# JackShDr/InfluentialRS

Hardware: NVIDIA B200
Metric: IRN influence-path generation throughput @1M items (higher is better)
Workload: dtype f32

## Files before the change

### influentialrs_b200/csrc/decoder_chain_tc.cu

```cuda
#include "tc_common.cuh"
#include "qkv_image.cuh"

namespace irs {
namespace tcl {

using namespace irs::tc;

constexpr int BM = 128, D = 128, F = 256;
constexpr int RING = 4;
constexpr uint32_t UNIT_BYTES = 16384, UNIT_HALF = 8192;
constexpr uint32_t A_LBO = BM * 16;
constexpr uint32_t SBO = 128;
constexpr uint32_t OFF_P = 0;
constexpr uint32_t OFF_Q = 65536;
constexpr uint32_t OFF_RING = 131072;
constexpr uint32_t OFF_VEC = OFF_RING + RING * UNIT_BYTES;
constexpr int V_BO = 0, V_G1 = 128, V_B1 = 256, V_C2 = 384, V_G2 = 512, V_B2 = 640, V_BF1 = 768, V_BF2 = 1024,
              V_G3 = 1152, V_B3 = 1280, V_BIN = 1408, V_TOTAL = 1792;
constexpr uint32_t OFF_XCH = OFF_VEC + V_TOTAL * 4;
constexpr uint32_t OFF_BARS = OFF_XCH + 3 * 2 * 128 * 8;
enum Bars { B_FULL = 0, B_EMPTY = 4, B_A0 = 8, B_D1 = 9, B_A1 = 10, B_D2 = 11, B_A2 = 12 , B_D3 = 16,
            B_A3 = 17, B_D4 = 18, B_COUNT = 20 };
constexpr uint32_t OFF_TMEM = OFF_BARS + B_COUNT * 8;
constexpr uint32_t SMEM_BYTES = OFF_TMEM + 16;
constexpr int EPI_WARPS = 8, EPI_THREADS = EPI_WARPS * 32;
constexpr int LOAD_WARPS = 2;
constexpr int WARP_LOAD0 = 8, WARP_PROD = 10, WARP_MMA = 11;
constexpr int THREADS = 12 * 32;
constexpr int UNITS_BODY = 20;
constexpr int UNITS_QKV = 12;
constexpr uint32_t T_H = 0, T_Y = 256, T_D3 = 384;

struct Params {
  const float* attn;
  const float* x;
  float* x_out;
  float* qkv_out;
  uint8_t* qkv_images;
  int L, mask_mode;
  int qkv_only;
  const uint4* wstream;
  const float* vec[11];
  float eps1, eps2, eps3;
  int64_t R; int64_t n_tiles; int n_units;
  int* error_flag;
  long long* timeline;
};

struct UnitDesc { int mat, n0, k0, kind; };
__host__ __device__ inline UnitDesc unit_desc(int u) {
  UnitDesc d;
  if (u < 4) { d.mat = 0; d.n0 = 0; d.k0 = 32 * u; d.kind = 0; }
  else if (u < 12) { d.mat = 1; d.n0 = 0; d.k0 = 16 * (u - 4); d.kind = 2; }
  else if (u < 20) { d.mat = 2; d.n0 = 0; d.k0 = 32 * (u - 12); d.kind = 0; }
  else if (u < 28) { d.mat = 3; d.n0 = 0; d.k0 = 16 * (u - 20); d.kind = 2; }
  else { d.mat = 3; d.n0 = 256; d.k0 = 32 * (u - 28); d.kind = 0; }
  return d;
}

__global__ void __launch_bounds__(256)
prepare_chain_kernel(const float* __restrict__ Wo, const float* __restrict__ W1, const float* __restrict__ W2,
                     const float* __restrict__ Win, int n_units, uint4* __restrict__ out) {
  const int total = n_units * 1024;
  for (int idx = blockIdx.x * blockDim.x + threadIdx.x; idx < total; idx += gridDim.x * blockDim.x) {
    const int u = idx >> 10, w = idx & 1023;
    const int part = w >> 9, rem = w & 511;
    const UnitDesc ud = unit_desc(u);
    int slab, row;
    if (ud.kind == 0) { slab = rem >> 7; row = rem & 127; } else { slab = rem >> 8; row = rem & 255; }
    const float* W; int ldw;
    switch (ud.mat) { case 0: W = Wo; ldw = D; break; case 1: W = W1; ldw = D; break; case 2: W = W2; ldw = F; break;
                      default: W = Win; ldw = D; break; }
    const float* src = W + (int64_t)(ud.n0 + row) * ldw + ud.k0 + slab * 8;
    float x[8];
#pragma unroll
    for (int e = 0; e < 8; ++e) x[e] = src[e];
    uint4 hi, lo;
    split8(x, hi, lo);
    out[idx] = part ? lo : hi;
  }
}

__device__ __forceinline__ void ldg256_nc(const float* p, float (&a)[8]) {
  asm volatile("ld.global.nc.L1::no_allocate.v8.f32 {%0,%1,%2,%3,%4,%5,%6,%7}, [%8];"
               : "=f"(a[0]), "=f"(a[1]), "=f"(a[2]), "=f"(a[3]), "=f"(a[4]), "=f"(a[5]), "=f"(a[6]), "=f"(a[7]) : "l"(p));
}
__device__ __forceinline__ void ldg256(const float* p, float (&a)[8]) {
  asm volatile("ld.global.L1::no_allocate.v8.f32 {%0,%1,%2,%3,%4,%5,%6,%7}, [%8];"
               : "=f"(a[0]), "=f"(a[1]), "=f"(a[2]), "=f"(a[3]), "=f"(a[4]), "=f"(a[5]), "=f"(a[6]), "=f"(a[7]) : "l"(p) : "memory");
}
__device__ __forceinline__ void stg256(float* p, const float* a) {
  asm volatile("st.global.L1::no_allocate.v8.f32 [%0], {%1,%2,%3,%4,%5,%6,%7,%8};"
               :: "l"(p), "f"(a[0]), "f"(a[1]), "f"(a[2]), "f"(a[3]), "f"(a[4]), "f"(a[5]), "f"(a[6]), "f"(a[7]) : "memory");
}
__device__ __forceinline__ void stg128(void* p, const uint4& v) {
  asm volatile("st.global.L1::no_allocate.v4.b32 [%0], {%1,%2,%3,%4};" :: "l"(p), "r"(v.x), "r"(v.y), "r"(v.z), "r"(v.w) : "memory");
}
__device__ __forceinline__ void prefetch_l2_bulk(const void* p, uint32_t bytes) {
  asm volatile("cp.async.bulk.prefetch.L2.global [%0], %1;" :: "l"(p), "r"(bytes) : "memory");
}

template <int KSTEPS>
__device__ __forceinline__ void mma_unit(uint32_t d_tmem, uint32_t a_hi, uint32_t a_lo, uint32_t b_stage, uint32_t b_lbo,
                                         uint32_t idesc, bool first) {
#pragma unroll
  for (int kk = 0; kk < KSTEPS; ++kk) {
    const uint64_t ah = make_desc(a_hi + (uint32_t)(2 * kk) * A_LBO, A_LBO, SBO);
    const uint64_t al = make_desc(a_lo + (uint32_t)(2 * kk) * A_LBO, A_LBO, SBO);
    const uint64_t bh = make_desc(b_stage + (uint32_t)(2 * kk) * b_lbo, b_lbo, SBO);
    const uint64_t bl = make_desc(b_stage + UNIT_HALF + (uint32_t)(2 * kk) * b_lbo, b_lbo, SBO);
    tc_mma_bf16(d_tmem, al, bh, idesc, (first && kk == 0) ? 0u : 1u);
    tc_mma_bf16(d_tmem, ah, bl, idesc, 1u);
    tc_mma_bf16(d_tmem, ah, bh, idesc, 1u);
  }
}

#define IRS_TL(role, idx)                                                                         \
  do {                                                                                            \
    if (p.timeline && blockIdx.x == 0 && it < 8 && lane == 0)                                     \
      p.timeline[(it * 3 + (role)) * 32 + (idx)] = clock64();                                     \
  } while (0)

__device__ __forceinline__ void pair_barrier(int quad) {
  asm volatile("bar.sync %0, 64;" :: "r"(1 + quad) : "memory");
}

__device__ __forceinline__ float2 ln_pair_stats(float (&t)[64], float2* mine, const float2* other, int quad, float eps) {
  float s[4] = {0.f, 0.f, 0.f, 0.f}, q[4] = {0.f, 0.f, 0.f, 0.f};
#pragma unroll
  for (int j = 0; j < 64; ++j) s[j & 3] += t[j];
  const float m = ((s[0] + s[1]) + (s[2] + s[3])) * (1.0f / 64.0f);
#pragma unroll
  for (int j = 0; j < 64; ++j) {
    t[j] -= m;
    q[j & 3] = fmaf(t[j], t[j], q[j & 3]);
  }
  const float qs = (q[0] + q[1]) + (q[2] + q[3]);
  *mine = make_float2(m, qs);
  pair_barrier(quad);
  const float2 o = *other;
  const float delta = o.x - m;
  const float mean = 0.5f * (m + o.x);
  const float rstd = rsqrtf(fmaf(32.f * delta, delta, qs + o.y) * (1.0f / (float)D) + eps);
  return make_float2(rstd, (m - mean) * rstd);
}

__global__ void __launch_bounds__(THREADS, 1)
decoder_chain_kernel(const Params p) {
  extern __shared__ __align__(128) uint8_t smem[];
  const uint32_t sbase = smem_u32(smem);
  const int tid = threadIdx.x, warp = tid >> 5, lane = tid & 31;
  auto bar = [&](int i) { return sbase + OFF_BARS + 8u * (uint32_t)i; };
  volatile uint32_t* tmem_holder = reinterpret_cast<volatile uint32_t*>(smem + OFF_TMEM);
  float* vecs = reinterpret_cast<float*>(smem + OFF_VEC);
  const bool with_qkv = (p.qkv_out != nullptr) || (p.qkv_images != nullptr);
  const bool qkv_only = p.qkv_only != 0;

  if (tid == 0) {
    for (int s = 0; s < RING; ++s) { mbar_init(bar(B_FULL + s), 1); mbar_init(bar(B_EMPTY + s), 1); }
    mbar_init(bar(B_A0), LOAD_WARPS);
    mbar_init(bar(B_D1), 1);
    mbar_init(bar(B_A1), EPI_THREADS);
    mbar_init(bar(B_D2), 1);
    for (int i = 0; i < 4; ++i) mbar_init(bar(B_A2 + i), EPI_THREADS);
    mbar_init(bar(B_D3), 1);
    mbar_init(bar(B_A3), EPI_THREADS);
    for (int i = 0; i < 2; ++i) mbar_init(bar(B_D4 + i), 1);
    asm volatile("fence.mbarrier_init.release.cluster;" ::: "memory");
  }
  if (warp == WARP_MMA) {
    asm volatile("tcgen05.alloc.cta_group::1.sync.aligned.shared::cta.b32 [%0], %1;" :: "r"(sbase + OFF_TMEM), "r"(512u) : "memory");
    asm volatile("tcgen05.relinquish_alloc_permit.cta_group::1.sync.aligned;" ::: "memory");
  }
  {
    const int vlen[11] = {128, 128, 128, 128, 128, 128, 256, 128, 128, 128, 384};
    int off = 0;
    const float qscale0 = 1.4426950408889634f / sqrtf((float)img::DH);
    for (int v = 0; v < 11; ++v) {
      for (int i = tid; i < vlen[v]; i += THREADS) {
        float x = p.vec[v] ? p.vec[v][i] : 0.f;
        if (v == 2 && p.vec[3]) x += p.vec[3][i];
        if (v == 10 && p.qkv_images && i < D) x *= qscale0;
        vecs[off + i] = x;
      }
      off += vlen[v];
    }
  }
  tc_fence_before();
  __syncthreads();
  tc_fence_after();
  const uint32_t tmem_base = *tmem_holder;
  const int64_t first_tile = blockIdx.x, tile_step = gridDim.x;

  if (warp >= WARP_LOAD0 && warp < WARP_LOAD0 + LOAD_WARPS) {
    const int lw = warp - WARP_LOAD0;
    const int r8 = lane & 7, sg = lane >> 3;
    const uint32_t a0_off = qkv_only ? OFF_P : OFF_Q;
    int it = 0;
    for (int64_t tile = first_tile; tile < p.n_tiles; tile += tile_step, ++it) {
      const int64_t r0 = tile * BM;
#pragma unroll 1
      for (int batch = 0; batch < 64 / LOAD_WARPS / 8; ++batch) {
        float v[8][8];
#pragma unroll
        for (int q = 0; q < 8; ++q) {
          const int qq = batch * 8 + q;
          const int row = (lw * (16 / LOAD_WARPS) + (qq >> 2)) * 8 + r8;
          const int slab = (qq & 3) * 4 + sg;
          if (r0 + row < p.R) ldg256_nc(p.attn + (r0 + row) * D + slab * 8, v[q]);
          else {
#pragma unroll
            for (int e = 0; e < 8; ++e) v[q][e] = 0.f;
          }
        }
        if (batch == 0 && lw == 0) IRS_TL(2, 0);
        if (batch == 0 && it > 0) mbar_wait(bar(qkv_only ? B_D4 + 1 : B_D3), (uint32_t)((it - 1) & 1), p.error_flag, 31);
        if (batch == 0 && lw == 0) IRS_TL(2, 1);
#pragma unroll
        for (int q = 0; q < 8; ++q) {
          const int qq = batch * 8 + q;
          const int row = (lw * (16 / LOAD_WARPS) + (qq >> 2)) * 8 + r8;
          const int slab = (qq & 3) * 4 + sg;
          uint4 hi, lo;
          split8(v[q], hi, lo);
          *reinterpret_cast<uint4*>(smem + a0_off + slab * A_LBO + row * 16) = hi;
          *reinterpret_cast<uint4*>(smem + a0_off + 32768 + slab * A_LBO + row * 16) = lo;
        }
      }
      asm volatile("fence.proxy.async.shared::cta;" ::: "memory");
      __syncwarp();
      if (lane == 0) mbar_arrive(bar(B_A0));
      if (lw == 0) IRS_TL(2, 2);
    }
  } else if (warp == WARP_PROD) {
    if (lane == 0) {
      int64_t g = 0;
      for (int64_t tile = first_tile; tile < p.n_tiles; tile += tile_step) {
        const int64_t nt = tile + tile_step;
        if (nt < p.n_tiles) {
          const int64_t rows = (p.R - nt * BM) < BM ? (p.R - nt * BM) : BM;
          if (p.x) prefetch_l2_bulk(p.x + nt * BM * D, (uint32_t)(rows * D * 4));
          prefetch_l2_bulk(p.attn + nt * BM * D, (uint32_t)(rows * D * 4));
        }
        for (int u = 0; u < p.n_units; ++u, ++g) {
          const int stage = (int)(g % RING);
          const uint32_t phase = (uint32_t)((g / RING) & 1);
          mbar_wait(bar(B_EMPTY + stage), phase ^ 1u, p.error_flag, 32);
          mbar_arrive_expect_tx(bar(B_FULL + stage), UNIT_BYTES);
          bulk_g2s(sbase + OFF_RING + stage * UNIT_BYTES, p.wstream + (int64_t)u * (UNIT_BYTES / 16), UNIT_BYTES, bar(B_FULL + stage));
        }
      }
    }
  } else if (warp == WARP_MMA) {
    if (lane == 0) {
      const uint32_t idesc128 = make_idesc_bf16(BM, 128), idesc256 = make_idesc_bf16(BM, 256);
      const uint32_t P_HI = sbase + OFF_P, P_LO = sbase + OFF_P + 32768, Q_HI = sbase + OFF_Q, Q_LO = sbase + OFF_Q + 32768;
      int64_t g = 0;
      auto next_unit = [&]() -> uint32_t {
        const int stage = (int)(g % RING);
        mbar_wait(bar(B_FULL + stage), (uint32_t)((g / RING) & 1), p.error_flag, 33);
        tc_fence_after();
        return sbase + OFF_RING + stage * UNIT_BYTES;
      };
      auto release_unit = [&]() { tc_commit(bar(B_EMPTY + (int)(g % RING))); ++g; };
      int it = 0;
      for (int64_t tile = first_tile; tile < p.n_tiles; tile += tile_step, ++it) {
        const uint32_t ph = (uint32_t)(it & 1);
        if (qkv_only) {
          mbar_wait(bar(B_A0), ph, p.error_flag, 34);
          if (it > 0) mbar_wait(bar(B_A1), (uint32_t)((it - 1) & 1), p.error_flag, 38);
          tc_fence_after();
          for (int u = 0; u < 8; ++u) {
            const uint32_t bs = next_unit();
            mma_unit<1>(tmem_base + T_H, P_HI + (uint32_t)(2 * u) * A_LBO, P_LO + (uint32_t)(2 * u) * A_LBO, bs, 4096u, idesc256, u == 0);
            release_unit();
          }
          tc_commit(bar(B_D4 + 0));
          for (int c = 0; c < 4; ++c) {
            const uint32_t bs = next_unit();
            mma_unit<2>(tmem_base + T_D3, P_HI + (uint32_t)(4 * c) * A_LBO, P_LO + (uint32_t)(4 * c) * A_LBO, bs, 2048u, idesc128, c == 0);
            release_unit();
          }
          tc_commit(bar(B_D4 + 1));
          continue;
        }
        IRS_TL(0, 0);
        mbar_wait(bar(B_A0), ph, p.error_flag, 34);
        tc_fence_after();
        IRS_TL(0, 1);
        for (int c = 0; c < 4; ++c) {
          const uint32_t bs = next_unit();
          mma_unit<2>(tmem_base + T_Y, Q_HI + (uint32_t)(4 * c) * A_LBO, Q_LO + (uint32_t)(4 * c) * A_LBO, bs, 2048u, idesc128, c == 0);
          release_unit();
        }
        tc_commit(bar(B_D1));
        IRS_TL(0, 2);
        mbar_wait(bar(B_A1), ph, p.error_flag, 35);
        tc_fence_after();
        IRS_TL(0, 3);
        for (int u = 0; u < 8; ++u) {
          const uint32_t bs = next_unit();
          mma_unit<1>(tmem_base + T_H, P_HI + (uint32_t)(2 * u) * A_LBO, P_LO + (uint32_t)(2 * u) * A_LBO, bs, 4096u, idesc256, u == 0);
          release_unit();
        }
        tc_commit(bar(B_D2));
        for (int j = 0; j < 4; ++j) {
          IRS_TL(0, 4 + 2 * j);
          mbar_wait(bar(B_A2 + j), ph, p.error_flag, 36);
          tc_fence_after();
          IRS_TL(0, 5 + 2 * j);
          const uint32_t slot = (j < 2 ? Q_HI : P_HI) + (uint32_t)(j & 1) * 32768u;
          for (int i = 0; i < 2; ++i) {
            const uint32_t bs = next_unit();
            mma_unit<2>(tmem_base + T_D3, slot + (uint32_t)(4 * i) * A_LBO, slot + 16384u + (uint32_t)(4 * i) * A_LBO, bs,
                        2048u, idesc128, j == 0 && i == 0);
            release_unit();
          }
        }
        tc_commit(bar(B_D3));
        IRS_TL(0, 12);
        mbar_wait(bar(B_A3), ph, p.error_flag, 37);
        tc_fence_after();
        IRS_TL(0, 13);
        if (with_qkv) {
          for (int u = 0; u < 8; ++u) {
            const uint32_t bs = next_unit();
            mma_unit<1>(tmem_base + T_H, P_HI + (uint32_t)(2 * u) * A_LBO, P_LO + (uint32_t)(2 * u) * A_LBO, bs, 4096u, idesc256, u == 0);
            release_unit();
          }
          tc_commit(bar(B_D4 + 0));
          IRS_TL(0, 14);
          for (int c = 0; c < 4; ++c) {
            const uint32_t bs = next_unit();
            mma_unit<2>(tmem_base + T_D3, P_HI + (uint32_t)(4 * c) * A_LBO, P_LO + (uint32_t)(4 * c) * A_LBO, bs, 2048u, idesc128, c == 0);
            release_unit();
          }
          tc_commit(bar(B_D4 + 1));
          IRS_TL(0, 15);
        }
      }
    }
  } else if (warp < EPI_WARPS) {
    const int quad = warp & 3, half = warp >> 2;
    const int row = quad * 32 + lane;
    const uint32_t tlane = tmem_base + (((uint32_t)(quad * 32)) << 16);
    float2* xch = reinterpret_cast<float2*>(smem + OFF_XCH);
    const int c0 = half * 64;
    auto e4_piece = [&](int64_t tile, int it, int piece) {
      const uint32_t ph = (uint32_t)(it & 1);
      const int64_t r = tile * BM + row;
      const bool row_ok = r < p.R;
      float* qo = p.qkv_out ? p.qkv_out + (row_ok ? r : 0) * (3 * D) : nullptr;
      const int bb = (int)(r / p.L), ll = (int)(r - (int64_t)bb * p.L);
      const int n_chunks = (p.L + 31) / 32;
      const int qs = img::q_slot(n_chunks, ll);
      const uint32_t q_off = img::OFF_Q + (uint32_t)(qs / BM) * img::Q_TILE + (uint32_t)(qs % BM) * 16u;
      const uint32_t kv_off = (uint32_t)img::kv_col(p.mask_mode == IRS_MASK_PIM, p.L, ll) * 16u;
      uint8_t* item0 = p.qkv_images ? p.qkv_images + (int64_t)bb * (D / img::DH) * img::ITEM_BYTES : nullptr;
      const float qscale = 1.4426950408889634f / sqrtf((float)img::DH);
      {
      mbar_wait(bar(B_D4 + piece), ph, p.error_flag, 45);
      tc_fence_after();
      if (warp == 0) IRS_TL(1, 13 + 2 * piece);
      const int ncol = piece == 0 ? 128 : 64;
      const int col0 = piece == 0 ? half * 128 : 256 + half * 64;
      const uint32_t tcol = piece == 0 ? (T_H + (uint32_t)half * 128u) : (T_D3 + (uint32_t)half * 64u);
      auto emit = [&](const uint32_t (&v)[32], int ch) {
        float o32[32];
        const float sc = (p.qkv_images && col0 + ch * 32 < D) ? qscale : 1.0f;
#pragma unroll
        for (int j = 0; j < 32; ++j) o32[j] = fmaf(__uint_as_float(v[j]), sc, vecs[V_BIN + col0 + ch * 32 + j]);
        if (qo) {
          if (row_ok) {
#pragma unroll
            for (int q = 0; q < 4; ++q) stg256(qo + col0 + ch * 32 + q * 8, &o32[q * 8]);
          }
        } else if (row_ok) {
          const int c = col0 + ch * 32;
          const int which = c >> 7, head = (c & 127) >> 5;
          uint8_t* dst = item0 + (int64_t)head * img::ITEM_BYTES + (which == 0 ? q_off : (which == 1 ? img::OFF_K : img::OFF_V) + kv_off);
          const uint32_t lbo = which == 0 ? img::Q_LBO : img::K_LBO, part = which == 0 ? img::Q_PART : img::K_PART;
#pragma unroll
          for (int s8 = 0; s8 < 4; ++s8) {
            uint4 hi, lo;
            split8(*reinterpret_cast<float(*)[8]>(&o32[s8 * 8]), hi, lo);
            stg128(dst + s8 * lbo, hi);
            stg128(dst + part + s8 * lbo, lo);
          }
        }
      };
      {
        const int nch = ncol / 32;
        uint32_t va[32], vb[32];
        tc_ld32(tlane + tcol, va);
#pragma unroll 1
        for (int ch = 0; ch < nch; ch += 2) {
          tc_wait_ld();
          if (ch + 1 < nch) tc_ld32(tlane + tcol + (ch + 1) * 32, vb);
          emit(va, ch);
          if (ch + 1 < nch) {
            tc_wait_ld();
            if (ch + 2 < nch) tc_ld32(tlane + tcol + (ch + 2) * 32, va);
            emit(vb, ch + 1);
          }
        }
      }
      if (warp == 0) IRS_TL(1, 14 + 2 * piece);
      }
    };
    int it = 0;
    for (int64_t tile = first_tile; tile < p.n_tiles; tile += tile_step, ++it) {
      const uint32_t ph = (uint32_t)(it & 1);
      const int64_t r = tile * BM + row;
      const bool row_ok = r < p.R;
      if (!qkv_only) {
      float t[64];
      {
        const float* xrow = p.x + (row_ok ? r : 0) * D + c0;
#pragma unroll
        for (int q = 0; q < 8; ++q) {
          if (row_ok) ldg256(xrow + q * 8, *reinterpret_cast<float(*)[8]>(&t[q * 8]));
          else {
#pragma unroll
            for (int e = 0; e < 8; ++e) t[q * 8 + e] = 0.f;
          }
        }
      }
      if (warp == 0) IRS_TL(1, 0);
      mbar_wait(bar(B_D1), ph, p.error_flag, 41);
      tc_fence_after();
      if (warp == 0) IRS_TL(1, 1);
#pragma unroll
      for (int ch = 0; ch < 2; ++ch) {
        uint32_t v[32];
        tc_ld32(tlane + T_Y + c0 + ch * 32, v);
        tc_wait_ld();
#pragma unroll
        for (int j = 0; j < 32; ++j) {
          t[ch * 32 + j] = __uint_as_float(v[j]) + vecs[V_BO + c0 + ch * 32 + j] + t[ch * 32 + j];
        }
      }
      const float2 st1 = ln_pair_stats(t, &xch[(0 * 2 + half) * 128 + row], &xch[(0 * 2 + (half ^ 1)) * 128 + row],
                                       quad, p.eps1);
#pragma unroll
      for (int j = 0; j < 64; ++j) {
        const int n = c0 + j;
        t[j] = fmaf(fmaf(t[j], st1.x, st1.y), vecs[V_G1 + n], vecs[V_B1 + n]);
      }
      const float2 st2 = ln_pair_stats(t, &xch[(1 * 2 + half) * 128 + row], &xch[(1 * 2 + (half ^ 1)) * 128 + row],
                                       quad, p.eps2);
#pragma unroll
      for (int ch = 0; ch < 2; ++ch) {
        uint32_t v[32];
#pragma unroll
        for (int j = 0; j < 32; ++j) {
          const int n = c0 + ch * 32 + j;
          const float y = fmaf(fmaf(t[ch * 32 + j], st2.x, st2.y), vecs[V_G2 + n], vecs[V_B2 + n]);
          t[ch * 32 + j] = y;
          v[j] = __float_as_uint(y);
        }
        tc_st32(tlane + T_Y + c0 + ch * 32, v);
#pragma unroll
        for (int s8 = 0; s8 < 4; ++s8) {
          uint4 hi, lo;
          split8(*reinterpret_cast<float(*)[8]>(&t[ch * 32 + s8 * 8]), hi, lo);
          const uint32_t o = (uint32_t)(half * 8 + ch * 4 + s8) * A_LBO + (uint32_t)row * 16u;
          *reinterpret_cast<uint4*>(smem + OFF_P + o) = hi;
          *reinterpret_cast<uint4*>(smem + OFF_P + 32768 + o) = lo;
        }
      }
      tc_wait_st();
      asm volatile("fence.proxy.async.shared::cta;" ::: "memory");
      tc_fence_before();
      mbar_arrive(bar(B_A1));
      if (warp == 0) IRS_TL(1, 2);
      if (with_qkv && it > 0) e4_piece(tile - tile_step, it - 1, 1);
      mbar_wait(bar(B_D2), ph, p.error_flag, 42);
      tc_fence_after();
#pragma unroll 1
      for (int j = 0; j < 4; ++j) {
        uint32_t v[32];
        tc_ld32(tlane + T_H + 64u * (uint32_t)j + 32u * (uint32_t)half, v);
        if (warp == 0) IRS_TL(1, 3 + 2 * j);
        uint8_t* slot = smem + (j < 2 ? OFF_Q : OFF_P) + (j & 1) * 32768;
        tc_wait_ld();
#pragma unroll
        for (int s8 = 0; s8 < 4; ++s8) {
          float x8[8];
#pragma unroll
          for (int e = 0; e < 8; ++e)
            x8[e] = fmaxf(__uint_as_float(v[s8 * 8 + e]) + vecs[V_BF1 + j * 64 + half * 32 + s8 * 8 + e], 0.f);
          uint4 hi, lo;
          split8(x8, hi, lo);
          const uint32_t o = (uint32_t)(half * 4 + s8) * A_LBO + (uint32_t)row * 16u;
          *reinterpret_cast<uint4*>(slot + o) = hi;
          *reinterpret_cast<uint4*>(slot + 16384 + o) = lo;
        }
        asm volatile("fence.proxy.async.shared::cta;" ::: "memory");
        tc_fence_before();
        mbar_arrive(bar(B_A2 + j));
        if (warp == 0) IRS_TL(1, 4 + 2 * j);
      }
      mbar_wait(bar(B_D3), ph, p.error_flag, 44);
      tc_fence_after();
      if (warp == 0) IRS_TL(1, 11);
#pragma unroll
      for (int ch = 0; ch < 2; ++ch) {
        uint32_t v[32], y[32];
        tc_ld32(tlane + T_D3 + c0 + ch * 32, v);
        tc_ld32(tlane + T_Y + c0 + ch * 32, y);
        tc_wait_ld();
#pragma unroll
        for (int j = 0; j < 32; ++j) {
          t[ch * 32 + j] = __uint_as_float(v[j]) + vecs[V_BF2 + c0 + ch * 32 + j] + __uint_as_float(y[j]);
        }
      }
      const float2 st3 = ln_pair_stats(t, &xch[(2 * 2 + half) * 128 + row], &xch[(2 * 2 + (half ^ 1)) * 128 + row],
                                       quad, p.eps3);
      float* xo = p.x_out + (row_ok ? r : 0) * D + c0;
#pragma unroll
      for (int ch = 0; ch < 2; ++ch) {
#pragma unroll
        for (int j = 0; j < 32; ++j) {
          const int n = c0 + ch * 32 + j;
          t[ch * 32 + j] = fmaf(fmaf(t[ch * 32 + j], st3.x, st3.y), vecs[V_G3 + n], vecs[V_B3 + n]);
        }
        if (row_ok) {
#pragma unroll
          for (int q = 0; q < 4; ++q) stg256(xo + ch * 32 + q * 8, &t[ch * 32 + q * 8]);
        }
        if (with_qkv) {
#pragma unroll
          for (int s8 = 0; s8 < 4; ++s8) {
            uint4 hi, lo;
            split8(*reinterpret_cast<float(*)[8]>(&t[ch * 32 + s8 * 8]), hi, lo);
            const uint32_t o = (uint32_t)(half * 8 + ch * 4 + s8) * A_LBO + (uint32_t)row * 16u;
            *reinterpret_cast<uint4*>(smem + OFF_P + o) = hi;
            *reinterpret_cast<uint4*>(smem + OFF_P + 32768 + o) = lo;
          }
        }
      }
      if (with_qkv) asm volatile("fence.proxy.async.shared::cta;" ::: "memory");
      tc_fence_before();
      mbar_arrive(bar(B_A3));
      if (warp == 0) IRS_TL(1, 12);
      }
      if (qkv_only) {
        e4_piece(tile, it, 0);
        e4_piece(tile, it, 1);
        tc_fence_before();
        mbar_arrive(bar(B_A1));
      } else if (with_qkv) {
        e4_piece(tile, it, 0);
      }
      tc_fence_before();
    }
    if (!qkv_only && with_qkv && it > 0) e4_piece(first_tile + (int64_t)(it - 1) * tile_step, it - 1, 1);
    tc_fence_before();
  }

  tc_fence_before();
  __syncthreads();
  if (warp == WARP_MMA) {
    tc_fence_after();
    asm volatile("tcgen05.dealloc.cta_group::1.sync.aligned.b32 %0, %1;" :: "r"(tmem_base), "r"(512u) : "memory");
  }
}

}
}

using namespace irs;

static long long* g_chain_timeline = nullptr;

extern "C" void irs_decoder_chain_debug_timeline(long long* buf) { g_chain_timeline = buf; }

extern "C" int irs_decoder_chain_supported(int d, int ffn) { return (d == tcl::D && ffn == tcl::F) ? 1 : 0; }

extern "C" size_t irs_decoder_chain_prepared_bytes(int d, int ffn, int with_in_proj) {
  if (!irs_decoder_chain_supported(d, ffn)) return 0;
  return (size_t)(tcl::UNITS_BODY + (with_in_proj ? tcl::UNITS_QKV : 0)) * tcl::UNIT_BYTES;
}

extern "C" int irs_decoder_chain_prepare_weights(const float* Wo, const float* W1, const float* W2, const float* Win,
                                                 int d, int ffn, void* prepared, void* stream) {
  if (!Wo || !W1 || !W2 || !prepared) return IRS_E_BADARG;
  if (!irs_decoder_chain_supported(d, ffn)) return IRS_E_SHAPE;
  const int n_units = tcl::UNITS_BODY + (Win ? tcl::UNITS_QKV : 0);
  tcl::prepare_chain_kernel<<<64, 256, 0, (cudaStream_t)stream>>>(Wo, W1, W2, Win, n_units, (uint4*)prepared);
  IRS_LAUNCHED();
  return 0;
}

static int chain_launch(tcl::Params& p, int64_t R, int* error_flag, void* stream) {
  p.R = R; p.n_tiles = ceil_div(R, tcl::BM);
  p.error_flag = error_flag;
  p.timeline = g_chain_timeline;
  static bool configured = false;
  if (!configured) {
    IRS_CUDA(cudaFuncSetAttribute(tcl::decoder_chain_kernel, cudaFuncAttributeMaxDynamicSharedMemorySize, (int)tcl::SMEM_BYTES));
    configured = true;
  }
  const unsigned grid = (unsigned)(p.n_tiles < kNumSMs ? p.n_tiles : kNumSMs);
  tcl::decoder_chain_kernel<<<grid, tcl::THREADS, tcl::SMEM_BYTES, (cudaStream_t)stream>>>(p);
  IRS_LAUNCHED();
  return 0;
}

extern "C" int irs_decoder_chain_tc(const float* attn, const float* x, const void* prepared,
                                    const float* bo, const float* g1, const float* b1, const float* c2,
                                    const float* g2, const float* b2, const float* bf1, const float* bf2,
                                    const float* g3, const float* b3, const float* bin,
                                    float eps1, float eps2, float eps3,
                                    float* x_out, float* qkv_out, void* qkv_images, int L, int mask_mode,
                                    int64_t R, int d, int ffn, int* error_flag, void* stream) {
  if (!attn || !x || !prepared || !x_out || !g1 || !b1 || !g2 || !b2 || !g3 || !b3) return IRS_E_BADARG;
  if (R < 0 || (qkv_out && qkv_images)) return IRS_E_BADARG;
  if (R == 0) return 0;
  if (!irs_decoder_chain_supported(d, ffn)) return IRS_E_SHAPE;
  if (qkv_images && (L <= 128 || L > irs::img::KEYS - 1 || R % L != 0 || mask_mode < 0 || mask_mode > 2)) return IRS_E_SHAPE;
  if (((uintptr_t)attn & 31) || ((uintptr_t)x & 31) || ((uintptr_t)x_out & 31) || ((uintptr_t)qkv_out & 31) ||
      ((uintptr_t)qkv_images & 15) || ((uintptr_t)prepared & 15))
    return IRS_E_SHAPE;
  tcl::Params p = {};
  p.attn = attn; p.x = x; p.x_out = x_out; p.qkv_out = qkv_out; p.qkv_images = (uint8_t*)qkv_images;
  p.L = qkv_images ? L : 1; p.mask_mode = mask_mode; p.qkv_only = 0;
  p.wstream = (const uint4*)prepared;
  const float* vec[11] = {bo, g1, b1, c2, g2, b2, bf1, bf2, g3, b3, bin};
  for (int i = 0; i < 11; ++i) p.vec[i] = vec[i];
  p.eps1 = eps1; p.eps2 = eps2; p.eps3 = eps3;
  p.n_units = tcl::UNITS_BODY + ((qkv_out || qkv_images) ? tcl::UNITS_QKV : 0);
  return chain_launch(p, R, error_flag, stream);
}

extern "C" int irs_in_proj_images_tc(const float* x, const void* prepared_with_in_proj, const float* bin,
                                     void* qkv_images, int L, int mask_mode, int64_t R, int d,
                                     int* error_flag, void* stream) {
  if (!x || !prepared_with_in_proj || !qkv_images) return IRS_E_BADARG;
  if (R < 0) return IRS_E_BADARG;
  if (R == 0) return 0;
  if (d != tcl::D) return IRS_E_SHAPE;
  if (L <= 128 || L > irs::img::KEYS - 1 || R % L != 0 || mask_mode < 0 || mask_mode > 2) return IRS_E_SHAPE;
  if (((uintptr_t)x & 31) || ((uintptr_t)qkv_images & 15) || ((uintptr_t)prepared_with_in_proj & 15)) return IRS_E_SHAPE;
  tcl::Params p = {};
  p.attn = x; p.x = nullptr; p.x_out = nullptr; p.qkv_out = nullptr; p.qkv_images = (uint8_t*)qkv_images;
  p.L = L; p.mask_mode = mask_mode; p.qkv_only = 1;
  p.wstream = (const uint4*)prepared_with_in_proj + (size_t)tcl::UNITS_BODY * (tcl::UNIT_BYTES / 16);
  p.vec[10] = bin;
  p.n_units = tcl::UNITS_QKV;
  return chain_launch(p, R, error_flag, stream);
}
```

### influentialrs_b200/csrc/tc_common.cuh

```cuda
#pragma once
#include <cuda_bf16.h>
#include "common.cuh"

namespace irs {
namespace tc {

__device__ __forceinline__ uint32_t smem_u32(const void* p) { return (uint32_t)__cvta_generic_to_shared(p); }

__device__ __forceinline__ void mbar_init(uint32_t bar, uint32_t count) {
  asm volatile("mbarrier.init.shared::cta.b64 [%0], %1;" :: "r"(bar), "r"(count) : "memory");
}
__device__ __forceinline__ void mbar_arrive(uint32_t bar) {
  asm volatile("mbarrier.arrive.shared::cta.b64 _, [%0];" :: "r"(bar) : "memory");
}
__device__ __forceinline__ void mbar_arrive_expect_tx(uint32_t bar, uint32_t bytes) {
  asm volatile("mbarrier.arrive.expect_tx.shared::cta.b64 _, [%0], %1;" :: "r"(bar), "r"(bytes) : "memory");
}
__device__ __forceinline__ bool mbar_try_wait(uint32_t bar, uint32_t parity) {
  uint32_t ok;
  asm volatile("{\n\t.reg .pred p;\n\t"
               "mbarrier.try_wait.parity.shared::cta.b64 p, [%1], %2, %3;\n\t"
               "selp.u32 %0, 1, 0, p;\n\t}"
               : "=r"(ok) : "r"(bar), "r"(parity), "r"(0x989680u) : "memory");
  return ok != 0;
}
__device__ __forceinline__ void mbar_wait(uint32_t bar, uint32_t parity, int* error_flag, int code) {
  if (mbar_try_wait(bar, parity)) return;
  const long long t0 = clock64();
  while (!mbar_try_wait(bar, parity)) {
    if (clock64() - t0 > 4000000000ll) {
      if (error_flag) atomicExch(error_flag, code);
      __threadfence_system();
      __trap();
    }
  }
}
__device__ __forceinline__ void bulk_g2s(uint32_t dst, const void* src, uint32_t bytes, uint32_t bar) {
  asm volatile("cp.async.bulk.shared::cluster.global.mbarrier::complete_tx::bytes [%0], [%1], %2, [%3];"
               :: "r"(dst), "l"(src), "r"(bytes), "r"(bar) : "memory");
}
__device__ __forceinline__ void tc_fence_before() { asm volatile("tcgen05.fence::before_thread_sync;" ::: "memory"); }
__device__ __forceinline__ void tc_fence_after() { asm volatile("tcgen05.fence::after_thread_sync;" ::: "memory"); }
__device__ __forceinline__ void tc_commit(uint32_t bar) {
  asm volatile("tcgen05.commit.cta_group::1.mbarrier::arrive::one.shared::cluster.b64 [%0];" :: "r"(bar) : "memory");
}
__device__ __forceinline__ void tc_mma_bf16(uint32_t d_tmem, uint64_t a_desc, uint64_t b_desc, uint32_t idesc, uint32_t accumulate) {
  asm volatile("{\n\t.reg .pred p;\n\t"
               "setp.ne.b32 p, %4, 0;\n\t"
               "tcgen05.mma.cta_group::1.kind::f16 [%0], %1, %2, %3, p;\n\t}"
               :: "r"(d_tmem), "l"(a_desc), "l"(b_desc), "r"(idesc), "r"(accumulate) : "memory");
}
__device__ __forceinline__ void tc_ld32(uint32_t taddr, uint32_t (&v)[32]) {
  asm volatile("tcgen05.ld.sync.aligned.32x32b.x32.b32 "
               "{%0,%1,%2,%3,%4,%5,%6,%7,%8,%9,%10,%11,%12,%13,%14,%15,"
               "%16,%17,%18,%19,%20,%21,%22,%23,%24,%25,%26,%27,%28,%29,%30,%31}, [%32];"
               : "=r"(v[0]), "=r"(v[1]), "=r"(v[2]), "=r"(v[3]), "=r"(v[4]), "=r"(v[5]), "=r"(v[6]), "=r"(v[7]),
                 "=r"(v[8]), "=r"(v[9]), "=r"(v[10]), "=r"(v[11]), "=r"(v[12]), "=r"(v[13]), "=r"(v[14]), "=r"(v[15]),
                 "=r"(v[16]), "=r"(v[17]), "=r"(v[18]), "=r"(v[19]), "=r"(v[20]), "=r"(v[21]), "=r"(v[22]), "=r"(v[23]),
                 "=r"(v[24]), "=r"(v[25]), "=r"(v[26]), "=r"(v[27]), "=r"(v[28]), "=r"(v[29]), "=r"(v[30]), "=r"(v[31])
               : "r"(taddr));
}
__device__ __forceinline__ void tc_wait_ld() { asm volatile("tcgen05.wait::ld.sync.aligned;" ::: "memory"); }
__device__ __forceinline__ void tc_st32(uint32_t taddr, const uint32_t (&v)[32]) {
  asm volatile("tcgen05.st.sync.aligned.32x32b.x32.b32 [%0], "
               "{%1,%2,%3,%4,%5,%6,%7,%8,%9,%10,%11,%12,%13,%14,%15,%16,"
               "%17,%18,%19,%20,%21,%22,%23,%24,%25,%26,%27,%28,%29,%30,%31,%32};"
               :: "r"(taddr),
                  "r"(v[0]), "r"(v[1]), "r"(v[2]), "r"(v[3]), "r"(v[4]), "r"(v[5]), "r"(v[6]), "r"(v[7]),
                  "r"(v[8]), "r"(v[9]), "r"(v[10]), "r"(v[11]), "r"(v[12]), "r"(v[13]), "r"(v[14]), "r"(v[15]),
                  "r"(v[16]), "r"(v[17]), "r"(v[18]), "r"(v[19]), "r"(v[20]), "r"(v[21]), "r"(v[22]), "r"(v[23]),
                  "r"(v[24]), "r"(v[25]), "r"(v[26]), "r"(v[27]), "r"(v[28]), "r"(v[29]), "r"(v[30]), "r"(v[31])
               : "memory");
}
__device__ __forceinline__ void tc_wait_st() { asm volatile("tcgen05.wait::st.sync.aligned;" ::: "memory"); }

__device__ __forceinline__ uint64_t make_desc(uint32_t saddr, uint32_t lbo, uint32_t sbo) {
  return (uint64_t)((saddr & 0x3FFFFu) >> 4) | ((uint64_t)((lbo >> 4) & 0x3FFFu) << 16) |
         ((uint64_t)((sbo >> 4) & 0x3FFFu) << 32) | (1ull << 46);
}
__host__ __device__ constexpr uint32_t make_idesc_bf16(int M, int N) {
  return (1u << 4) | (1u << 7) | (1u << 10) | ((uint32_t)(N >> 3) << 17) | ((uint32_t)(M >> 4) << 24);
}

__device__ __forceinline__ uint32_t pack_bf16x2(__nv_bfloat16 a, __nv_bfloat16 b) {
  return (uint32_t)__bfloat16_as_ushort(a) | ((uint32_t)__bfloat16_as_ushort(b) << 16);
}
__device__ __forceinline__ void split8(const float (&x)[8], uint4& hi, uint4& lo) {
  uint32_t hw[4], lw[4];
#pragma unroll
  for (int e = 0; e < 4; ++e) {
    const __nv_bfloat162 h2 = __floats2bfloat162_rn(x[2 * e], x[2 * e + 1]);
    const __nv_bfloat162 l2 = __floats2bfloat162_rn(x[2 * e] - __low2float(h2), x[2 * e + 1] - __high2float(h2));
    hw[e] = *reinterpret_cast<const uint32_t*>(&h2);
    lw[e] = *reinterpret_cast<const uint32_t*>(&l2);
  }
  hi = make_uint4(hw[0], hw[1], hw[2], hw[3]);
  lo = make_uint4(lw[0], lw[1], lw[2], lw[3]);
}


}
}
```

Measured before the change: 397,200.

## Double epilogue warps to sixteen, splitting each row's columns across four warps

Raises the epilogue from 8 to 16 warps so each thread handles 32 columns of a row instead of 64. LayerNorm statistics are now merged across four warps with a Chan-style equal-count combine through a larger shared-memory exchange and a 128-thread named barrier. TMEM loads switch to the x16 variant where the slices shrink. Tile indices also move from 64-bit to 32-bit. The aim is to shorten the per-tile epilogue critical path and lower register pressure, at the cost of more threads per CTA and more barrier traffic.

```diff
diff --git a/influentialrs_b200/csrc/decoder_chain_tc.cu b/influentialrs_b200/csrc/decoder_chain_tc.cu
--- a/influentialrs_b200/csrc/decoder_chain_tc.cu
+++ b/influentialrs_b200/csrc/decoder_chain_tc.cu
@@ -18,15 +18,15 @@
 constexpr int V_BO = 0, V_G1 = 128, V_B1 = 256, V_C2 = 384, V_G2 = 512, V_B2 = 640, V_BF1 = 768, V_BF2 = 1024,
               V_G3 = 1152, V_B3 = 1280, V_BIN = 1408, V_TOTAL = 1792;
 constexpr uint32_t OFF_XCH = OFF_VEC + V_TOTAL * 4;
-constexpr uint32_t OFF_BARS = OFF_XCH + 3 * 2 * 128 * 8;
+constexpr uint32_t OFF_BARS = OFF_XCH + 3 * 4 * 128 * 8;
 enum Bars { B_FULL = 0, B_EMPTY = 4, B_A0 = 8, B_D1 = 9, B_A1 = 10, B_D2 = 11, B_A2 = 12 , B_D3 = 16,
             B_A3 = 17, B_D4 = 18, B_COUNT = 20 };
 constexpr uint32_t OFF_TMEM = OFF_BARS + B_COUNT * 8;
 constexpr uint32_t SMEM_BYTES = OFF_TMEM + 16;
-constexpr int EPI_WARPS = 8, EPI_THREADS = EPI_WARPS * 32;
+constexpr int EPI_WARPS = 16, EPI_THREADS = EPI_WARPS * 32;
 constexpr int LOAD_WARPS = 2;
-constexpr int WARP_LOAD0 = 8, WARP_PROD = 10, WARP_MMA = 11;
-constexpr int THREADS = 12 * 32;
+constexpr int WARP_LOAD0 = 16, WARP_PROD = 18, WARP_MMA = 19;
+constexpr int THREADS = 20 * 32;
 constexpr int UNITS_BODY = 20;
 constexpr int UNITS_QKV = 12;
 constexpr uint32_t T_H = 0, T_Y = 256, T_D3 = 384;
@@ -42,7 +42,7 @@
   const uint4* wstream;
   const float* vec[11];
   float eps1, eps2, eps3;
-  int64_t R; int64_t n_tiles; int n_units;
+  int64_t R; int n_tiles; int n_units;
   int* error_flag;
   long long* timeline;
 };
@@ -121,28 +121,31 @@
       p.timeline[(it * 3 + (role)) * 32 + (idx)] = clock64();                                     \
   } while (0)
 
-__device__ __forceinline__ void pair_barrier(int quad) {
-  asm volatile("bar.sync %0, 64;" :: "r"(1 + quad) : "memory");
-}
-
-__device__ __forceinline__ float2 ln_pair_stats(float (&t)[64], float2* mine, const float2* other, int quad, float eps) {
+__device__ __forceinline__ void quad_barrier(int quad) {
+  asm volatile("bar.sync %0, 128;" :: "r"(1 + quad) : "memory");
+}
+
+__device__ __forceinline__ float2 chan_merge_equal(float2 a, float2 b, float half_n) {
+  const float delta = b.x - a.x;
+  return make_float2(0.5f * (a.x + b.x), fmaf(half_n * delta, delta, a.y + b.y));
+}
+
+__device__ __forceinline__ float2 ln_quad_stats(float (&t)[32], float2* xch, int qtr, int row, int quad, float eps) {
   float s[4] = {0.f, 0.f, 0.f, 0.f}, q[4] = {0.f, 0.f, 0.f, 0.f};
 #pragma unroll
-  for (int j = 0; j < 64; ++j) s[j & 3] += t[j];
-  const float m = ((s[0] + s[1]) + (s[2] + s[3])) * (1.0f / 64.0f);
-#pragma unroll
-  for (int j = 0; j < 64; ++j) {
+  for (int j = 0; j < 32; ++j) s[j & 3] += t[j];
+  const float m = ((s[0] + s[1]) + (s[2] + s[3])) * (1.0f / 32.0f);
+#pragma unroll
+  for (int j = 0; j < 32; ++j) {
     t[j] -= m;
     q[j & 3] = fmaf(t[j], t[j], q[j & 3]);
   }
-  const float qs = (q[0] + q[1]) + (q[2] + q[3]);
-  *mine = make_float2(m, qs);
-  pair_barrier(quad);
-  const float2 o = *other;
-  const float delta = o.x - m;
-  const float mean = 0.5f * (m + o.x);
-  const float rstd = rsqrtf(fmaf(32.f * delta, delta, qs + o.y) * (1.0f / (float)D) + eps);
-  return make_float2(rstd, (m - mean) * rstd);
+  xch[qtr * 128 + row] = make_float2(m, (q[0] + q[1]) + (q[2] + q[3]));
+  quad_barrier(quad);
+  const float2 st = chan_merge_equal(chan_merge_equal(xch[row], xch[128 + row], 16.f),
+                                     chan_merge_equal(xch[256 + row], xch[384 + row], 16.f), 32.f);
+  const float rstd = rsqrtf(st.y * (1.0f / (float)D) + eps);
+  return make_float2(rstd, (m - st.x) * rstd);
 }
 
 __global__ void __launch_bounds__(THREADS, 1)
@@ -190,15 +193,15 @@
   __syncthreads();
   tc_fence_after();
   const uint32_t tmem_base = *tmem_holder;
-  const int64_t first_tile = blockIdx.x, tile_step = gridDim.x;
+  const int first_tile = blockIdx.x, tile_step = gridDim.x;
 
   if (warp >= WARP_LOAD0 && warp < WARP_LOAD0 + LOAD_WARPS) {
     const int lw = warp - WARP_LOAD0;
     const int r8 = lane & 7, sg = lane >> 3;
     const uint32_t a0_off = qkv_only ? OFF_P : OFF_Q;
     int it = 0;
-    for (int64_t tile = first_tile; tile < p.n_tiles; tile += tile_step, ++it) {
-      const int64_t r0 = tile * BM;
+    for (int tile = first_tile; tile < p.n_tiles; tile += tile_step, ++it) {
+      const int64_t r0 = (int64_t)tile * BM;
 #pragma unroll 1
       for (int batch = 0; batch < 64 / LOAD_WARPS / 8; ++batch) {
         float v[8][8];
@@ -235,12 +238,12 @@
   } else if (warp == WARP_PROD) {
     if (lane == 0) {
       int64_t g = 0;
-      for (int64_t tile = first_tile; tile < p.n_tiles; tile += tile_step) {
-        const int64_t nt = tile + tile_step;
+      for (int tile = first_tile; tile < p.n_tiles; tile += tile_step) {
+        const int nt = tile + tile_step;
         if (nt < p.n_tiles) {
-          const int64_t rows = (p.R - nt * BM) < BM ? (p.R - nt * BM) : BM;
-          if (p.x) prefetch_l2_bulk(p.x + nt * BM * D, (uint32_t)(rows * D * 4));
-          prefetch_l2_bulk(p.attn + nt * BM * D, (uint32_t)(rows * D * 4));
+          const int64_t rows = (p.R - (int64_t)nt * BM) < BM ? (p.R - (int64_t)nt * BM) : BM;
+          if (p.x) prefetch_l2_bulk(p.x + (int64_t)nt * BM * D, (uint32_t)(rows * D * 4));
+          prefetch_l2_bulk(p.attn + (int64_t)nt * BM * D, (uint32_t)(rows * D * 4));
         }
         for (int u = 0; u < p.n_units; ++u, ++g) {
           const int stage = (int)(g % RING);
@@ -264,7 +267,7 @@
       };
       auto release_unit = [&]() { tc_commit(bar(B_EMPTY + (int)(g % RING))); ++g; };
       int it = 0;
-      for (int64_t tile = first_tile; tile < p.n_tiles; tile += tile_step, ++it) {
+      for (int tile = first_tile; tile < p.n_tiles; tile += tile_step, ++it) {
         const uint32_t ph = (uint32_t)(it & 1);
         if (qkv_only) {
           mbar_wait(bar(B_A0), ph, p.error_flag, 34);
@@ -341,14 +344,15 @@
       }
     }
   } else if (warp < EPI_WARPS) {
-    const int quad = warp & 3, half = warp >> 2;
+    const int quad = warp & 3, qtr = warp >> 2;
     const int row = quad * 32 + lane;
     const uint32_t tlane = tmem_base + (((uint32_t)(quad * 32)) << 16);
     float2* xch = reinterpret_cast<float2*>(smem + OFF_XCH);
-    const int c0 = half * 64;
-    auto e4_piece = [&](int64_t tile, int it, int piece) {
+    const int c0 = qtr * 32;
+    const uint32_t tcols = tlane + (uint32_t)c0;
+    auto e4_piece = [&](int tile, int it, int piece) {
       const uint32_t ph = (uint32_t)(it & 1);
-      const int64_t r = tile * BM + row;
+      const int64_t r = (int64_t)tile * BM + row;
       const bool row_ok = r < p.R;
       float* qo = p.qkv_out ? p.qkv_out + (row_ok ? r : 0) * (3 * D) : nullptr;
       const int bb = (int)(r / p.L), ll = (int)(r - (int64_t)bb * p.L);
@@ -362,63 +366,62 @@
       mbar_wait(bar(B_D4 + piece), ph, p.error_flag, 45);
       tc_fence_after();
       if (warp == 0) IRS_TL(1, 13 + 2 * piece);
-      const int ncol = piece == 0 ? 128 : 64;
-      const int col0 = piece == 0 ? half * 128 : 256 + half * 64;
-      const uint32_t tcol = piece == 0 ? (T_H + (uint32_t)half * 128u) : (T_D3 + (uint32_t)half * 64u);
-      auto emit = [&](const uint32_t (&v)[32], int ch) {
-        float o32[32];
-        const float sc = (p.qkv_images && col0 + ch * 32 < D) ? qscale : 1.0f;
-#pragma unroll
-        for (int j = 0; j < 32; ++j) o32[j] = fmaf(__uint_as_float(v[j]), sc, vecs[V_BIN + col0 + ch * 32 + j]);
+      const int ncol = piece == 0 ? 64 : 32;
+      const int col0 = piece == 0 ? qtr * 64 : 256 + qtr * 32;
+      const uint32_t tcol = piece == 0 ? (T_H + (uint32_t)qtr * 64u) : (T_D3 + (uint32_t)qtr * 32u);
+      auto emit = [&](const uint32_t (&v)[16], int ch) {
+        const int c = col0 + ch * 16;
+        float o16[16];
+        const float sc = (p.qkv_images && c < D) ? qscale : 1.0f;
+#pragma unroll
+        for (int j = 0; j < 16; ++j) o16[j] = fmaf(__uint_as_float(v[j]), sc, vecs[V_BIN + c + j]);
         if (qo) {
           if (row_ok) {
 #pragma unroll
-            for (int q = 0; q < 4; ++q) stg256(qo + col0 + ch * 32 + q * 8, &o32[q * 8]);
+            for (int q = 0; q < 2; ++q) stg256(qo + c + q * 8, &o16[q * 8]);
           }
         } else if (row_ok) {
-          const int c = col0 + ch * 32;
           const int which = c >> 7, head = (c & 127) >> 5;
-          uint8_t* dst = item0 + (int64_t)head * img::ITEM_BYTES + (which == 0 ? q_off : (which == 1 ? img::OFF_K : img::OFF_V) + kv_off);
           const uint32_t lbo = which == 0 ? img::Q_LBO : img::K_LBO, part = which == 0 ? img::Q_PART : img::K_PART;
-#pragma unroll
-          for (int s8 = 0; s8 < 4; ++s8) {
+          uint8_t* dst = item0 + (int64_t)head * img::ITEM_BYTES + (which == 0 ? q_off : (which == 1 ? img::OFF_K : img::OFF_V) + kv_off) +
+                         (uint32_t)((c & 31) >> 3) * lbo;
+#pragma unroll
+          for (int s8 = 0; s8 < 2; ++s8) {
             uint4 hi, lo;
-            split8(*reinterpret_cast<float(*)[8]>(&o32[s8 * 8]), hi, lo);
+            split8(*reinterpret_cast<float(*)[8]>(&o16[s8 * 8]), hi, lo);
             stg128(dst + s8 * lbo, hi);
             stg128(dst + part + s8 * lbo, lo);
           }
         }
       };
       {
-        const int nch = ncol / 32;
-        uint32_t va[32], vb[32];
-        tc_ld32(tlane + tcol, va);
+        const int nch = ncol / 16;
+        uint32_t va[16], vb[16];
+        tc_ld16(tlane + tcol, va);
 #pragma unroll 1
         for (int ch = 0; ch < nch; ch += 2) {
           tc_wait_ld();
-          if (ch + 1 < nch) tc_ld32(tlane + tcol + (ch + 1) * 32, vb);
+          tc_ld16(tlane + tcol + (ch + 1) * 16, vb);
           emit(va, ch);
-          if (ch + 1 < nch) {
-            tc_wait_ld();
-            if (ch + 2 < nch) tc_ld32(tlane + tcol + (ch + 2) * 32, va);
-            emit(vb, ch + 1);
-          }
+          tc_wait_ld();
+          if (ch + 2 < nch) tc_ld16(tlane + tcol + (ch + 2) * 16, va);
+          emit(vb, ch + 1);
         }
       }
       if (warp == 0) IRS_TL(1, 14 + 2 * piece);
       }
     };
     int it = 0;
-    for (int64_t tile = first_tile; tile < p.n_tiles; tile += tile_step, ++it) {
+    for (int tile = first_tile; tile < p.n_tiles; tile += tile_step, ++it) {
       const uint32_t ph = (uint32_t)(it & 1);
-      const int64_t r = tile * BM + row;
+      const int64_t r = (int64_t)tile * BM + row;
       const bool row_ok = r < p.R;
       if (!qkv_only) {
-      float t[64];
+      float t[32];
       {
         const float* xrow = p.x + (row_ok ? r : 0) * D + c0;
 #pragma unroll
-        for (int q = 0; q < 8; ++q) {
+        for (int q = 0; q < 4; ++q) {
           if (row_ok) ldg256(xrow + q * 8, *reinterpret_cast<float(*)[8]>(&t[q * 8]));
           else {
 #pragma unroll
@@ -430,44 +433,38 @@
       mbar_wait(bar(B_D1), ph, p.error_flag, 41);
       tc_fence_after();
       if (warp == 0) IRS_TL(1, 1);
-#pragma unroll
-      for (int ch = 0; ch < 2; ++ch) {
+      {
         uint32_t v[32];
-        tc_ld32(tlane + T_Y + c0 + ch * 32, v);
+        tc_ld32(tcols + T_Y, v);
         tc_wait_ld();
 #pragma unroll
-        for (int j = 0; j < 32; ++j) {
-          t[ch * 32 + j] = __uint_as_float(v[j]) + vecs[V_BO + c0 + ch * 32 + j] + t[ch * 32 + j];
-        }
-      }
-      const float2 st1 = ln_pair_stats(t, &xch[(0 * 2 + half) * 128 + row], &xch[(0 * 2 + (half ^ 1)) * 128 + row],
-                                       quad, p.eps1);
-#pragma unroll
-      for (int j = 0; j < 64; ++j) {
+        for (int j = 0; j < 32; ++j) t[j] = __uint_as_float(v[j]) + vecs[V_BO + c0 + j] + t[j];
+      }
+      const float2 st1 = ln_quad_stats(t, xch, qtr, row, quad, p.eps1);
+#pragma unroll
+      for (int j = 0; j < 32; ++j) {
         const int n = c0 + j;
         t[j] = fmaf(fmaf(t[j], st1.x, st1.y), vecs[V_G1 + n], vecs[V_B1 + n]);
       }
-      const float2 st2 = ln_pair_stats(t, &xch[(1 * 2 + half) * 128 + row], &xch[(1 * 2 + (half ^ 1)) * 128 + row],
-                                       quad, p.eps2);
-#pragma unroll
-      for (int ch = 0; ch < 2; ++ch) {
+      const float2 st2 = ln_quad_stats(t, xch + 4 * 128, qtr, row, quad, p.eps2);
+      {
         uint32_t v[32];
 #pragma unroll
         for (int j = 0; j < 32; ++j) {
-          const int n = c0 + ch * 32 + j;
-          const float y = fmaf(fmaf(t[ch * 32 + j], st2.x, st2.y), vecs[V_G2 + n], vecs[V_B2 + n]);
-          t[ch * 32 + j] = y;
+          const int n = c0 + j;
+          const float y = fmaf(fmaf(t[j], st2.x, st2.y), vecs[V_G2 + n], vecs[V_B2 + n]);
+          t[j] = y;
           v[j] = __float_as_uint(y);
         }
-        tc_st32(tlane + T_Y + c0 + ch * 32, v);
-#pragma unroll
-        for (int s8 = 0; s8 < 4; ++s8) {
-          uint4 hi, lo;
-          split8(*reinterpret_cast<float(*)[8]>(&t[ch * 32 + s8 * 8]), hi, lo);
-          const uint32_t o = (uint32_t)(half * 8 + ch * 4 + s8) * A_LBO + (uint32_t)row * 16u;
-          *reinterpret_cast<uint4*>(smem + OFF_P + o) = hi;
-          *reinterpret_cast<uint4*>(smem + OFF_P + 32768 + o) = lo;
-        }
+        tc_st32(tcols + T_Y, v);
+      }
+#pragma unroll
+      for (int s8 = 0; s8 < 4; ++s8) {
+        uint4 hi, lo;
+        split8(*reinterpret_cast<float(*)[8]>(&t[s8 * 8]), hi, lo);
+        const uint32_t o = (uint32_t)(qtr * 4 + s8) * A_LBO + (uint32_t)row * 16u;
+        *reinterpret_cast<uint4*>(smem + OFF_P + o) = hi;
+        *reinterpret_cast<uint4*>(smem + OFF_P + 32768 + o) = lo;
       }
       tc_wait_st();
       asm volatile("fence.proxy.async.shared::cta;" ::: "memory");
@@ -479,20 +476,20 @@
       tc_fence_after();
 #pragma unroll 1
       for (int j = 0; j < 4; ++j) {
-        uint32_t v[32];
-        tc_ld32(tlane + T_H + 64u * (uint32_t)j + 32u * (uint32_t)half, v);
+        uint32_t v[16];
+        tc_ld16(tlane + T_H + 64u * (uint32_t)j + 16u * (uint32_t)qtr, v);
         if (warp == 0) IRS_TL(1, 3 + 2 * j);
         uint8_t* slot = smem + (j < 2 ? OFF_Q : OFF_P) + (j & 1) * 32768;
         tc_wait_ld();
 #pragma unroll
-        for (int s8 = 0; s8 < 4; ++s8) {
+        for (int s8 = 0; s8 < 2; ++s8) {
           float x8[8];
 #pragma unroll
           for (int e = 0; e < 8; ++e)
-            x8[e] = fmaxf(__uint_as_float(v[s8 * 8 + e]) + vecs[V_BF1 + j * 64 + half * 32 + s8 * 8 + e], 0.f);
+            x8[e] = fmaxf(__uint_as_float(v[s8 * 8 + e]) + vecs[V_BF1 + j * 64 + qtr * 16 + s8 * 8 + e], 0.f);
           uint4 hi, lo;
           split8(x8, hi, lo);
-          const uint32_t o = (uint32_t)(half * 4 + s8) * A_LBO + (uint32_t)row * 16u;
+          const uint32_t o = (uint32_t)(qtr * 2 + s8) * A_LBO + (uint32_t)row * 16u;
           *reinterpret_cast<uint4*>(slot + o) = hi;
           *reinterpret_cast<uint4*>(slot + 16384 + o) = lo;
         }
@@ -504,43 +501,36 @@
       mbar_wait(bar(B_D3), ph, p.error_flag, 44);
       tc_fence_after();
       if (warp == 0) IRS_TL(1, 11);
-#pragma unroll
-      for (int ch = 0; ch < 2; ++ch) {
+      {
         uint32_t v[32], y[32];
-        tc_ld32(tlane + T_D3 + c0 + ch * 32, v);
-        tc_ld32(tlane + T_Y + c0 + ch * 32, y);
+        tc_ld32(tcols + T_D3, v);
+        tc_ld32(tcols + T_Y, y);
         tc_wait_ld();
 #pragma unroll
-        for (int j = 0; j < 32; ++j) {
-          t[ch * 32 + j] = __uint_as_float(v[j]) + vecs[V_BF2 + c0 + ch * 32 + j] + __uint_as_float(y[j]);
-        }
-      }
-      const float2 st3 = ln_pair_stats(t, &xch[(2 * 2 + half) * 128 + row], &xch[(2 * 2 + (half ^ 1)) * 128 + row],
-                                       quad, p.eps3);
-      float* xo = p.x_out + (row_ok ? r : 0) * D + c0;
-#pragma unroll
-      for (int ch = 0; ch < 2; ++ch) {
-#pragma unroll
-        for (int j = 0; j < 32; ++j) {
-          const int n = c0 + ch * 32 + j;
-          t[ch * 32 + j] = fmaf(fmaf(t[ch * 32 + j], st3.x, st3.y), vecs[V_G3 + n], vecs[V_B3 + n]);
-        }
-        if (row_ok) {
-#pragma unroll
-          for (int q = 0; q < 4; ++q) stg256(xo + ch * 32 + q * 8, &t[ch * 32 + q * 8]);
-        }
-        if (with_qkv) {
-#pragma unroll
-          for (int s8 = 0; s8 < 4; ++s8) {
-            uint4 hi, lo;
-            split8(*reinterpret_cast<float(*)[8]>(&t[ch * 32 + s8 * 8]), hi, lo);
-            const uint32_t o = (uint32_t)(half * 8 + ch * 4 + s8) * A_LBO + (uint32_t)row * 16u;
-            *reinterpret_cast<uint4*>(smem + OFF_P + o) = hi;
-            *reinterpret_cast<uint4*>(smem + OFF_P + 32768 + o) = lo;
-          }
-        }
-      }
-      if (with_qkv) asm volatile("fence.proxy.async.shared::cta;" ::: "memory");
+        for (int j = 0; j < 32; ++j) t[j] = __uint_as_float(v[j]) + vecs[V_BF2 + c0 + j] + __uint_as_float(y[j]);
+      }
+      const float2 st3 = ln_quad_stats(t, xch + 8 * 128, qtr, row, quad, p.eps3);
+#pragma unroll
+      for (int j = 0; j < 32; ++j) {
+        const int n = c0 + j;
+        t[j] = fmaf(fmaf(t[j], st3.x, st3.y), vecs[V_G3 + n], vecs[V_B3 + n]);
+      }
+      if (row_ok) {
+        float* xo = p.x_out + r * D + c0;
+#pragma unroll
+        for (int q = 0; q < 4; ++q) stg256(xo + q * 8, &t[q * 8]);
+      }
+      if (with_qkv) {
+#pragma unroll
+        for (int s8 = 0; s8 < 4; ++s8) {
+          uint4 hi, lo;
+          split8(*reinterpret_cast<float(*)[8]>(&t[s8 * 8]), hi, lo);
+          const uint32_t o = (uint32_t)(qtr * 4 + s8) * A_LBO + (uint32_t)row * 16u;
+          *reinterpret_cast<uint4*>(smem + OFF_P + o) = hi;
+          *reinterpret_cast<uint4*>(smem + OFF_P + 32768 + o) = lo;
+        }
+        asm volatile("fence.proxy.async.shared::cta;" ::: "memory");
+      }
       tc_fence_before();
       mbar_arrive(bar(B_A3));
       if (warp == 0) IRS_TL(1, 12);
@@ -555,7 +545,7 @@
       }
       tc_fence_before();
     }
-    if (!qkv_only && with_qkv && it > 0) e4_piece(first_tile + (int64_t)(it - 1) * tile_step, it - 1, 1);
+    if (!qkv_only && with_qkv && it > 0) e4_piece(first_tile + (it - 1) * tile_step, it - 1, 1);
     tc_fence_before();
   }
 
@@ -594,7 +584,7 @@
 }
 
 static int chain_launch(tcl::Params& p, int64_t R, int* error_flag, void* stream) {
-  p.R = R; p.n_tiles = ceil_div(R, tcl::BM);
+  p.R = R; p.n_tiles = (int)ceil_div(R, tcl::BM);
   p.error_flag = error_flag;
   p.timeline = g_chain_timeline;
   static bool configured = false;
diff --git a/influentialrs_b200/csrc/tc_common.cuh b/influentialrs_b200/csrc/tc_common.cuh
--- a/influentialrs_b200/csrc/tc_common.cuh
+++ b/influentialrs_b200/csrc/tc_common.cuh
@@ -60,6 +60,13 @@
                  "=r"(v[24]), "=r"(v[25]), "=r"(v[26]), "=r"(v[27]), "=r"(v[28]), "=r"(v[29]), "=r"(v[30]), "=r"(v[31])
                : "r"(taddr));
 }
+__device__ __forceinline__ void tc_ld16(uint32_t taddr, uint32_t (&v)[16]) {
+  asm volatile("tcgen05.ld.sync.aligned.32x32b.x16.b32 "
+               "{%0,%1,%2,%3,%4,%5,%6,%7,%8,%9,%10,%11,%12,%13,%14,%15}, [%16];"
+               : "=r"(v[0]), "=r"(v[1]), "=r"(v[2]), "=r"(v[3]), "=r"(v[4]), "=r"(v[5]), "=r"(v[6]), "=r"(v[7]),
+                 "=r"(v[8]), "=r"(v[9]), "=r"(v[10]), "=r"(v[11]), "=r"(v[12]), "=r"(v[13]), "=r"(v[14]), "=r"(v[15])
+               : "r"(taddr));
+}
 __device__ __forceinline__ void tc_wait_ld() { asm volatile("tcgen05.wait::ld.sync.aligned;" ::: "memory"); }
 __device__ __forceinline__ void tc_st32(uint32_t taddr, const uint32_t (&v)[32]) {
   asm volatile("tcgen05.st.sync.aligned.32x32b.x32.b32 [%0], "
```

Result: no change. 393,400, median of 6 (-1.0%).
